# skovaka/UNCALLED

Measured on NVIDIA H100. Metric: reads/sec mapped (E. coli, 4k-sample reads) at 1/2/4/8 H100 vs CPU ref, higher is better.
Workload: dtype f32/f64 events, u32 FM index

## Files before the change

### uncalled_b200/csrc/unc_device.cuh

```cuda
#pragma once
#include "unc_warp.cuh"

typedef uint8_t u8;
typedef uint16_t u16;
typedef uint32_t u32;
typedef int32_t i32;
typedef uint64_t u64;

#define UNC_NKMER 1024
#define UNC_KMASK 0x3FFu
#define UNC_SEED_LEN 22u
#define UNC_NGEN 24u
#define UNC_PATH_MASK 0x3FFFFFu
#define UNC_PATH_TAIL 0x200000u
#define UNC_INVALID 0x80000000u
#define UNC_BLK 32u


struct DevIndex {
    const uint4 *bwt;
    const u32 *sa;
    const u32 *sa_full;
    const uint2 *kmer_range;
    const float *lv_mean, *lv_var2, *lognorm;
// ... 742 lines not shown
#else
#define K2_DYN_FUSE 0u
#endif
#ifdef K2_LEAN_B
#define K2_DYN_PER_CHUNK (44u + K2_DYN_FUSE)
#else
#define K2_DYN_PER_CHUNK (24u + K2_DYN_FUSE)
#endif
#define K2_SMEM_BYTES(maxp) (sizeof(K2Shared) + 16 + (size_t) (((maxp) + 31) / 32) * K2_DYN_PER_CHUNK + 32 + K2_V2_DYN_BYTES)
struct K2Tables {
    uint2 kmer_range[UNC_NKMER];
    float thresh[64];
};
struct K2V2 {
    K2V2Tab t;
    u32 kcnt[UNC_NKMER];
    u32 koff[UNC_NKMER];
    u32 kagg[UNC_NKMER];
    u32 fresh_cand[32], fresh_mask[32], fresh_before[32];
    u32 grab[2];
    u32 n_units;
    u16 mfirst[K2V2_MAX_MERGED];
#if defined(UNC_PHASE_TIMING) && !defined(UNC_EMUL)
    u32 pt_dur[4][K2_MAXSEG];
#endif
};
struct K2Shared {
    K2Tables tb;
    float probs[UNC_NKMER];
    u32 flags[32];
    u32 flags_prev[32];
#ifdef K2_OCC_STAGE
    uint4 occ_stage[K2_MAXSEG * 32 * 5];
#endif
    u32 hist_cur[K2_RB * K2_MAXSEG];
    u32 hist_next[K2_RB * K2_MAXSEG];
    uint2 *agg;
    u64 *pre;
    u32 *bcnt, *ecnt;
    u32 *cmb;
    K2V2 v2;
    unsigned char *v2_stage;
#ifdef K2_DFUSE
    u64 *agg2;
#endif
    u32 bc[8];
    u32 scan_tmp[32];
    u32 n_rows[2];
    u32 verdict[2];
    u32 wk_overflow;
    u32 wl_cnt;
    u32 cnt_blocks, cnt_steps;
    u32 tot_children[2], tot_sources[2];
#ifdef K2_TRK_INLINE
    u32 trk_state[24];
#endif
};

#include "unc_pdqsort.cuh"
#ifdef UNC_EMUL
static unsigned long g_emu_tie_stats[2];
#endif

UNC_DEV void k2_wk_exscan_bins(K2Shared *sh, u32 *src, u32 *dst, u32 wt, u32 nwt) {
    const u32 n = K2_RB * K2_MAXSEG;
    const u32 per = (n + nwt - 1) / nwt;
    const u32 lo = wt * per < n ? wt * per : n, hi = lo + per < n ? lo + per : n;
    u32 sum = 0;
    for (u32 j = lo; j < hi; j++) sum += src[j];
    u32 wtot, woff = w_exscan(sum, &wtot);
    if (w_lane() == 31) sh->scan_tmp[wt >> 5] = wtot;
    c_sync_sub(1, (int) nwt);
#ifdef K2_SCAN2
    u32 run;
    {
        u32 v = (u32) w_lane() < (nwt >> 5) ? sh->scan_tmp[w_lane()] : 0, t;
        u32 e = w_exscan(v, &t);
        run = w_shfl(e, (int) (wt >> 5)) + woff;
    }
#else
    if (wt < 32) {
        u32 v = wt < (nwt >> 5) ? sh->scan_tmp[wt] : 0, t;
        u32 e = w_exscan(v, &t);
        sh->scan_tmp[wt] = e;
    }
    c_sync_sub(1, (int) nwt);
    u32 run = sh->scan_tmp[wt >> 5] + woff;
#endif
    for (u32 j = lo; j < hi; j++) {
        u32 cnt = src[j];
        dst[j] = run;
        src[j] = 0;
        run += cnt;
    }
    c_sync_sub(1, (int) nwt);
}

UNC_DEV void write_source(uint4 *rec, uint2 *hist_e, u32 idx, u32 st, u32 en, u32 kmer, float prob) {
    rec[(size_t) idx * 2] = make_uint4(st, en, kmer | (1u << 16), 1u);
    rec[(size_t) idx * 2 + 1] = make_uint4(f2u(prob), f2u(prob), 0u, 0u);
    hist_e[idx] = make_uint2(f2u(prob), 0xFFFFFFFFu);
}

UNC_DEV u32 unc_event_to_bp(u32 evt_i, bool last, float mean_event_len, float bp_per_samp) {
    float v = f_add(f_mul(f_mul((float) evt_i, mean_event_len), bp_per_samp), (float) (last ? 4 : 0));
    return f_to_u32_x86(v);
// ... 1154 lines not shown
        trk_state_load(sh->trk_state, t1);
        const u32 verdict = sh->trk_state[21], final_event = sh->trk_state[22];
        if (STREAM) {
            DevMapState *ms = B.mstate + B.chan[r];
            ms->t_nb = t1.nb; ms->t_n_alloc = t1.n_alloc; ms->t_n_live = t1.n_live; ms->t_n_lens = t1.n_lens;
            ms->t_top1 = t1.top1; ms->t_top2 = t1.top2; ms->t_overflow = t1.overflow; ms->t_len_sum = t1.len_sum;
            ms->t_max_map[0] = t1.max_map.ren_start; ms->t_max_map[1] = t1.max_map.evt_en; ms->t_max_map[2] = t1.max_map.ref_st;
            ms->t_max_map[3] = t1.max_map.ren_end; ms->t_max_map[4] = t1.max_map.evt_st; ms->t_max_map[5] = t1.max_map.total_len;
            ms->event_i = final_event;
            ms->started = 1;
        }
        unc_k2_write_record(ix, p, B, sh, r, t1, verdict, final_event, ((u64) sh->trk_state[20] << 32) | sh->trk_state[19]);
    }
#else
    if (tid < 32) unc_k2_tracker<STREAM>(ix, p, B, W, sh, r, n_first, n_limit,
                                                              K2_V2_ACTIVE && !EXACT ? (uint4 *) sh->hist_next : nullptr, K2_RB * K2_MAXSEG / 4u);
#ifndef K2_V1
    else if (!EXACT) unc_k2_workers_v2<STREAM, FLAGS>(ix, p, B, W, sh, r, n_first, n_limit);
#endif
    else unc_k2_workers<STREAM, EXACT, FLAGS>(ix, p, B, W, sh, r, n_first, n_limit, epoch_io);
#endif
    c_sync();
    if (STREAM && tid < 32) B.mstate[B.chan[r]].flags[tid] = sh->flags[tid];
    if (!STREAM && FLAGS && B.flags_out && tid < 32) B.flags_out[(size_t) r * 32 + tid] = sh->flags[tid];
}

UNC_DEV bool unc_event0_cand(const DevIndex &ix, const DevParams &p, const DevBatch &B, u32 r, u32 k) {
    if (B.n_events[r] == 0 || p.max_events == 0) return false;
    const float event = f_add(f_mul(B.scale[r], B.events[(size_t) r * B.ev_stride]), B.shift[r]);
    const uint2 kr = ix.kmer_range[k];
    return unc_match_prob(event, d_ldg(ix.lv_mean + k), d_ldg(ix.lv_var2 + k), d_ldg(ix.lognorm + k)) >= ix.thresh[0] &&
           kr.x <= kr.y;
}

UNC_DEV DevWork unc_work_slot(const DevWork &W0, const DevWorkStrides &S, size_t slot) {
    DevWork W;
    W.paths = W0.paths + slot * S.paths;
    W.hist = W0.hist + slot * S.hist;
    W.wlist = W0.wlist + slot * S.cks;
    W.ckey = W0.ckey + slot * S.ckey;
    W.cks = W0.cks + slot * S.cks;
    W.elist = W0.elist + slot * S.elist;
    W.order = W0.order + slot * S.order;
    W.rlist = W0.rlist + slot * S.rlist;
    W.clu = W0.clu + slot * S.clu;
    W.dir = W0.dir + slot * S.dir;
    W.max_blocks = W0.max_blocks;
    W.rl_cap = W0.rl_cap;
    return W;
}

template <bool EXACT = false, bool FLAGS = false>
UNC_DEV void unc_k2_cta_main(const DevIndex &ix, const DevParams &p, const DevBatch &B, const DevWork &W, K2Shared *sh) {
    unc_k2_cta_setup(ix, p, sh);
    u32 epoch = 0;
    for (;;) {
        if (c_tid() == 0) sh->bc[0] = d_atomic_add(B.queue, 1u);
        c_sync();
        u32 r = sh->bc[0];
        c_sync();
        if (r >= B.n_reads) break;
        unc_k2_map_read<false, EXACT, FLAGS>(ix, p, B, W, sh, r, &epoch);
    }
}

template <bool EXACT = false>
UNC_DEV void unc_k2_cta_main_stream(const DevIndex &ix, const DevParams &p, const DevBatch &B, const DevWork &W0,
                                    const DevWorkStrides &S, K2Shared *sh) {
    unc_k2_cta_setup(ix, p, sh);
    u32 epoch = 0;
    for (;;) {
        if (c_tid() == 0) sh->bc[0] = d_atomic_add(B.queue, 1u);
        c_sync();
        u32 r = sh->bc[0];
        c_sync();
        if (r >= B.n_reads) break;
        const DevWork W = unc_work_slot(W0, S, B.chan[r]);
        unc_k2_map_read<true, EXACT, true>(ix, p, B, W, sh, r, &epoch);
    }
}
```

### uncalled_b200/csrc/unc_k2v2.cuh

```cuda
#pragma once

#define K2V2_STAGE_BYTES (K2_CH_SLOTS * 8u + K2_CH_SLOTS)


UNC_DEV void unc_occ2_build_block(const uint4 *bwt, u32 j, uint4 *out) {
    const uint4 *p = bwt + ((size_t) (j >> 1) << 2);
    const uint4 b0 = p[0], b1 = p[1];
    uint4 cnt = make_uint4(b0.x, b0.z, b1.x, b1.z);
    const uint4 lo = p[2], hi = p[3];
    if (j & 1u) {
        const u32 w[4] = {lo.x, lo.y, lo.z, lo.w};
        for (int i = 0; i < 4; i++) {
            const u32 h = w[i] >> 1, m = 0x55555555u;
            const u32 c3 = (u32) d_popc(h & w[i] & m), c2 = (u32) d_popc(h & ~w[i] & m), c1 = (u32) d_popc(~h & w[i] & m);
            cnt.x += 16u - c1 - c2 - c3; cnt.y += c1; cnt.z += c2; cnt.w += c3;
        }
    }
    out[(size_t) j * 2] = cnt;
    out[(size_t) j * 2 + 1] = (j & 1u) ? hi : lo;
}

UNC_DEV void unc_occ2_all(const uint4 cnt, const uint4 sym, u32 p, u32 o[4]) {
    u32 c1 = 0, c2 = 0, c3 = 0;
#pragma unroll
// ... 108 lines not shown
UNC_DEV K2V2Walk k2v2_walk(const uint4 cur, u32 nx, u32 ny, bool a, bool has_next, bool head, bool first, bool use_carry,
                           u32 carry_mx, bool prob_ok, uint2 kr, u32 *mx_last) {
    const int lane = w_lane();
    K2V2Walk r;
    r.dup = has_next && nx == cur.x && ny == cur.y;
    u32 mx = a ? cur.y : 0u;
    bool hd = head || !a;
    for (int d = 1; d < 32; d <<= 1) {
        const u32 omx = w_shfl_up(mx, d), ohd = w_shfl_up(hd ? 1u : 0u, d);
        if (lane >= d && !hd) { mx = omx > mx ? omx : mx; hd = ohd != 0; }
    }
    if (use_carry) mx = mx > carry_mx ? mx : carry_mx;
    *mx_last = w_shfl(mx, 31);
    r.begin_v = a && first && prob_ok && kr.x <= cur.x - 1u;
    r.as = mx + 1u;
    r.ae = has_next ? nx - 1u : kr.y;
    r.after_v = a && !r.dup && prob_ok && r.as <= r.ae;
    r.seed = a && !r.dup && (cur.w & 1u);
    r.m_b = w_ballot(r.begin_v); r.m_a = w_ballot(r.after_v); r.m_seed = w_ballot(r.seed);
    return r;
}

struct K2V2Pack {
    bool a;
    u32 bl;
    u32 start, pos, n;
};
UNC_DEV K2V2Pack k2v2_next_pack(u32 cnt, u32 P, u32 *remaining) {
    const int lane = w_lane();
    const int s = d_ffs(*remaining) - 1;
    const u32 Ps = w_shfl(P, s);
    const bool fits = ((*remaining >> lane) & 1u) && (P + cnt - Ps <= 32u);
    const u32 in_pack = w_ballot(fits);
    *remaining &= ~in_pack;
    const int e = 31 - d_clz(in_pack);
    const u32 T = w_shfl(P + cnt, e) - Ps;
    K2V2Pack k;
    k.a = (u32) lane < T;
    k.bl = (u32) s; k.start = 0;
    u32 m = in_pack;
    while (m) {
        const int b = d_ffs(m) - 1;
        m &= m - 1;
        const u32 sb = w_shfl(P, b) - Ps;
        if ((u32) lane >= sb) { k.bl = (u32) b; k.start = sb; }
    }
    k.pos = (u32) lane - k.start;
    k.n = w_shfl(cnt, (int) k.bl);
    return k;
}
UNC_DEV u32 k2v2_segmask(u32 start, u32 n) { return (n >= 32u ? 0xFFFFFFFFu : ((1u << n) - 1u)) << start; }

UNC_DEV u32 k2v2_slot(u32 rank) { return ((rank & 31u) << 5) | (rank >> 5); }

UNC_DEV u32 k2v2_grab(u32 *counter) {
    u32 g = 0;
    if (w_lane() == 0) g = s_atomic_add(counter, 1u);
    return w_shfl(g, 0);
}

UNC_DEV void k2v2_sort_small(uint4 *keys, u32 n, uint4 *sst) {
    const int lane = w_lane();
    const bool a = (u32) lane < n;
    uint4 k = make_uint4(0, 0, 0, 0);
    if (a) k = keys[lane];
    u32 rnk = 0;
    const u32 kf = k2v2_fkey(k.z), kr_ = k.w >> 14;
    for (u32 j = 0; j < n; j++) {
        const u32 jx = w_shfl(k.x, (int) j), jy = w_shfl(k.y, (int) j), jf = w_shfl(kf, (int) j), jr = w_shfl(kr_, (int) j);
        if (k2v2_less_pre(jx, jy, jf, jr, k.x, k.y, kf, kr_)) rnk++;
    }
    if (a) sst[rnk] = k;
    w_sync();
    if (a) keys[lane] = sst[lane];
    w_sync();
}

struct K2V2Emit {
    uint4 *next; uint2 *hist_e; u32 *onext; uint2 *rlist;
    u32 S0, nc, maxp, n_ended_rows, rl_cap, pos0;
    u32 src_before, seeds_before;
};
template <bool EMIT>
UNC_DEV u32 k2v2_walk_merged(const DevIndex &ix, K2Shared *sh, const uint4 *keys, u32 n, u32 moff, float source_prob,
                             const K2V2Emit &E, u32 *pend_steps, u32 *pend_blocks, uint4 *sst) {
    K2V2 *v2 = &sh->v2;
    const u32 lane = (u32) w_lane();
    u32 nsrc = 0, nseed = 0, prev_sub = 0xFFFFFFFFu, un_st = 1, un_en = 0;
  for (u32 g0 = 0; g0 < n; g0 += 32u) {
    const u32 cnt = n - g0 < 32u ? n - g0 : 32u;
    if (lane < cnt) sst[lane] = keys[g0 + lane];
    if (lane == 0 && g0 + cnt < n) sst[32] = keys[g0 + cnt];
    w_sync();
    if (lane == 0)
    for (u32 j = 0; j < cnt; j++) {
        const u32 i = g0 + j;
        const uint4 cur = sst[j];
        const u32 sub = (cur.w >> 6) & 0xFFu, kmer = v2->t.mk[moff + sub];
        const uint2 kr = sh->tb.kmer_range[kmer];
        const float pk = sh->probs[kmer];
        const bool ok = pk >= source_prob;
        if (sub != prev_sub) {
            if (!EMIT && v2->mfirst[moff + sub] == 0xFFFFu) v2->mfirst[moff + sub] = (u16) nsrc;
            if (ok) {
                if (kr.x <= cur.x - 1u) {
                    const u32 sidx = E.src_before + nsrc;
// ... 20 lines not shown
                src_en = nxt.x - 1u;
                if (un_st <= nxt.y) un_st = nxt.y + 1u;
            }
            if (src_st <= src_en) {
                const u32 sidx = E.src_before + nsrc;
                if (EMIT && E.nc + sidx < E.maxp) {
                    write_source(E.next, E.hist_e, E.S0 + E.nc + sidx, src_st, src_en, kmer, pk);
                    E.onext[E.nc + sidx] = E.S0 + E.nc + sidx;
                }
                nsrc++;
            }
        }
        if (cur.w & 1u) {
            if (EMIT) {
                d_atomic_or(&((u32 *) (E.next + (size_t) rec * 2))[3], 0x80000000u);
                const u32 ri = E.n_ended_rows + E.seeds_before + nseed;
                if (ri < E.rl_cap) E.rlist[ri] = make_uint2(ix.seq_len - unc_sa_lookup(ix, cur.x, pend_steps, pend_blocks), (cur.w >> 1) & 0x1Fu);
                else sh->wk_overflow = 1;
            }
            nseed++;
        }
    }
    w_sync();
  }
    return w_shfl(nsrc | (nseed << 16), 0);
}

UNC_DEV void k2v2_bucket_offsets(K2V2 *v2) {
    const u32 lane = (u32) w_lane();
    u32 sum = 0;
#pragma unroll 1
    for (u32 j = 0; j < 32; j++) sum += v2->kcnt[j * 32u + lane];
    u32 tot, run = w_exscan(sum, &tot);
#pragma unroll 1
    for (u32 j = 0; j < 32; j++) {
        const u32 sl = j * 32u + lane, v = v2->kcnt[sl];
        v2->koff[sl] = run;
        v2->kcnt[sl] = run;
        run += v;
    }
}

template <bool STREAM, bool FLAGS>
UNC_DEV void unc_k2_workers_v2(const DevIndex &ix, const DevParams &p, const DevBatch &B, const DevWork &W,
                               K2Shared *sh, u32 r, u32 n_first, u32 n_limit) {
    const int lane = w_lane();
    const u32 wt = (u32) c_tid() - 32u, nwt = (u32) c_nthreads() - 32u;
    const u32 ww = wt >> 5, nwk = nwt >> 5;
    const K2Tables *tb = &sh->tb;
    K2V2 *v2 = &sh->v2;
    const u32 maxp = p.max_paths;
    const u32 S0 = ((maxp + 31u) >> 5) * K2_CH_SLOTS;
    const size_t gen_recs = (size_t) S0 + maxp;
    const float scale = B.scale[r], shift = B.shift[r];
    const float *events = B.events + (size_t) r * B.ev_stride;
    const float source_prob = tb->thresh[0];
    u64 n_children = 0, n_sources = 0;
    u32 pend_children = 0, pend_sources = 0;
    u32 my_blocks = 0, my_steps = 0, pend_blocks = 0, pend_steps = 0;
    u32 prev_size = 0, gen = 0, event_i = n_first;
    if (STREAM) {
        const DevMapState *ms = B.mstate + B.chan[r];
        if (ms->started) { prev_size = ms->prev_size; gen = ms->gen; }
    }
    const u32 lt = w_lanemask_lt();
    uint2 *stage_r = (uint2 *) (sh->v2_stage + (size_t) ww * K2V2_STAGE_BYTES);
    u8 *stage_m = (u8 *) (stage_r + K2_CH_SLOTS);
    u32 *whist = sh->hist_cur + (size_t) ww * 256u;
    PT_DECL
    PT_WDECL

    for (; event_i < n_limit; event_i++) {
        PT_MARK(9)
        const float event = f_add(f_mul(scale, events[event_i - n_first]), shift);
        PT_MARK(7)

        if (FLAGS && wt < 32u) sh->flags_prev[wt] = sh->flags[wt];
        for (u32 k = wt; k < UNC_NKMER; k += nwt) {
            sh->probs[k] = unc_match_prob(event, d_ldg(ix.lv_mean + k), d_ldg(ix.lv_var2 + k), d_ldg(ix.lognorm + k));
            v2->kcnt[k] = 0; v2->kagg[k] = 0;
        }
        for (u32 j = ww; j < 32; j += nwk) {
            const u32 k = j * 32 + (u32) lane;
            const float pk = unc_match_prob(event, d_ldg(ix.lv_mean + k), d_ldg(ix.lv_var2 + k), d_ldg(ix.lognorm + k));
            const uint2 kr = tb->kmer_range[k];
            const u32 m = w_ballot(pk >= source_prob && kr.x <= kr.y);
            if (lane == 0) v2->fresh_cand[j] = m;
        }
        if (wt == 0) { v2->grab[0] = 0; v2->grab[1] = 0; v2->n_units = 0; }
        if (wt < K2V2_MAX_MERGED) v2->mfirst[wt] = 0xFFFFu;
        PT_MARK(0)
        c_sync_sub(1, (int) nwt);
        PT_FENCE
        PT_MARK(16)

        uint4 *prev = W.paths + (size_t) gen * gen_recs * 2, *next = W.paths + (size_t) (gen ^ 1u) * gen_recs * 2;
        uint2 *hist_e = W.hist + (size_t) (event_i % UNC_NGEN) * gen_recs;
        const u32 *oprev = W.order + (size_t) gen * maxp;
        u32 *onext = W.order + (size_t) (gen ^ 1u) * maxp;
        uint4 *ckA = W.ckey, *ckB = W.ckey + maxp, *cks = W.cks;
        uint2 *rlist = W.rlist + (size_t) (event_i & 1u) * W.rl_cap;

        const u32 nch_prev = (prev_size + 31u) >> 5;
        {
            u32 oi_n = UNC_INVALID, oi_nn = UNC_INVALID; uint4 q0_n = make_uint4(0, 0, 0, 0); uint2 q1_n = make_uint2(0, 0);
            if (ww < nch_prev) {
                const u32 pi = ww * 32u + (u32) lane;
                if (pi < prev_size) oi_n = oprev[pi];
                if (!(oi_n & UNC_INVALID)) { const uint4 *pr = prev + (size_t) oi_n * 2; q0_n = pr[0]; q1_n = *(const uint2 *) (pr + 1); }
            }
            if (ww + nwk < nch_prev) {
                const u32 pi = (ww + nwk) * 32u + (u32) lane;
                if (pi < prev_size) oi_nn = oprev[pi];
                if (!(oi_nn & UNC_INVALID)) d_prefetch(prev + (size_t) oi_nn * 2);
            }
            for (u32 c = ww; c < nch_prev; c += nwk) {
                const u32 oi = oi_n;
                const uint4 q0 = q0_n; const uint2 q1 = q1_n;
                const bool valid = !(oi & UNC_INVALID);
                oi_n = oi_nn;
                if (c + nwk < nch_prev && !(oi_n & UNC_INVALID)) {
                    const uint4 *pr = prev + (size_t) oi_n * 2;
                    q0_n = pr[0]; q1_n = *(const uint2 *) (pr + 1);
                }
                oi_nn = UNC_INVALID;
                if (c + 2u * nwk < nch_prev) {
                    const u32 pi = (c + 2u * nwk) * 32u + (u32) lane;
                    if (pi < prev_size) oi_nn = oprev[pi];
                    if (!(oi_nn & UNC_INVALID)) d_prefetch(prev + (size_t) oi_nn * 2);
                }
                const u32 st = q0.x, en = q0.y, kmer = q0.z & UNC_KMASK, plen = (q0.z >> 16) & 0xFFu, stays = (q0.z >> 24) & 0xFFu;
                const u32 moves = q0.w & UNC_PATH_MASK, sa_checked = q0.w >> 31;
                u32 want = 0, cmask = 0;
                if (valid) {
                    const float thr = tb->thresh[32 + d_clz(en - st + 1u)];
                    if (stays < p.max_consec_stay && sh->probs[kmer] >= thr) cmask = 1u;
#pragma unroll
                    for (u32 b = 0; b < 4; b++)
                        if (!(sh->probs[((kmer << 2) & UNC_KMASK) | b] < thr)) want |= 1u << b;
                }
                if (cmask) stage_r[(u32) lane * 5u] = make_uint2(st, en);
                if (want) {
                    const u32 k0 = st - 1u, l0 = en;
                    const u32 kk = k0 - (k0 >= ix.primary), ll = l0 - (l0 >= ix.primary);
                    const bool l_is_end = (l0 == ix.seq_len);
                    const uint4 *bk = ix.occ2 + ((size_t) (kk >> 6) << 1);
                    const uint4 kc = d_ldg(bk), ks = d_ldg(bk + 1);
                    uint4 lc = kc, ls = ks;
                    if (!l_is_end && (ll >> 6) != (kk >> 6)) {
                        const uint4 *bl = ix.occ2 + ((size_t) (ll >> 6) << 1);
                        lc = d_ldg(bl); ls = d_ldg(bl + 1);
                    }
                    pend_blocks += 1u + ((!l_is_end && (ll >> 7) != (kk >> 7)) ? 1u : 0u);
                    u32 ok[4], ol[4];
                    unc_occ2_all(kc, ks, kk & 63u, ok);
                    unc_occ2_all(lc, ls, ll & 63u, ol);
                    if (l_is_end) { ol[0] = ix.L2[1] - ix.L2[0]; ol[1] = ix.L2[2] - ix.L2[1]; ol[2] = ix.L2[3] - ix.L2[2]; ol[3] = ix.L2[4] - ix.L2[3]; }
// ... 34 lines not shown
                    const u32 pz = w_shfl(q0.z, L), pw = w_shfl(q0.w, L), pC = w_shfl(q1.y, L), poi = w_shfl(oi, L);
                    if (act) {
                        const u32 pk = pz & UNC_KMASK, ppl = (pz >> 16) & 0xFFu, pst = (pz >> 24) & 0xFFu;
                        const u32 ckm = j == 0 ? pk : (((pk << 2) & UNC_KMASK) | (j - 1u));
                        const float pb = sh->probs[ckm];
                        const u32 move = j > 0 ? 1u : 0u;
                        const u32 nlen = ppl + (ppl < UNC_SEED_LEN ? 1u : 0u);
                        u32 nmoves = (((pw & UNC_PATH_MASK) << 1) | move) & UNC_PATH_MASK;
                        const u32 nstays = move ? 0u : pst + 1u;
                        const float newC = f_add(u2f(pC), pb);
                        const u32 ci = c * K2_CH_SLOTS + t;
                        float sp = 0.0f;
                        bool seedable = false;
                        if (ppl == UNC_SEED_LEN) {
                            nmoves |= UNC_PATH_TAIL;
                            W.wlist[s_atomic_add(&sh->wl_cnt, 1u)] = make_uint4(ci, poi, f2u(newC), nmoves);
                        } else {
                            sp = f_div(newC, (float) nlen);
                            const u32 cmc = (u32) d_popc(nmoves);
                            seedable = nlen == UNC_SEED_LEN && sp >= p.min_seed_prob && rg.x == rg.y && (nmoves & 1u) &&
                                       (float) ((nlen - cmc) & 0xFFu) <= f_mul(p.max_stay_frac, 22.0f);
                        }
                        const u32 spb = f2u(sp);
                        next[(size_t) ci * 2] = make_uint4(rg.x, rg.y, ckm | (nlen << 16) | (nstays << 24), nmoves | (pw & 0x80000000u));
                        next[(size_t) ci * 2 + 1] = make_uint4(spb, f2u(newC), 0u, 0u);
                        hist_e[ci] = make_uint2(f2u(newC), poi);
                        cks[ci] = make_uint4(rg.x, rg.y, spb, ckm | (seedable ? 1u << 10 : 0u) | ((u32) d_popc(nmoves) << 11));
                        s_atomic_add(&v2->kcnt[v2->t.kslot[ckm]], 1u);
                    }
                }
                if (c + nwk < nch_prev && !(oi_n & UNC_INVALID)) {
                    const u32 k0n = q0_n.x - 1u;
                    d_prefetch(ix.occ2 + ((size_t) ((k0n - (k0n >= ix.primary)) >> 6) << 1));
                }
                w_sync();
            }
        }
        PT_MARK(1)
        c_sync_sub(1, (int) nwt);
        PT_FENCE
        PT_MARK(17)
        if (ww == 0) {
            {
                const u32 per = (nch_prev + 31u) >> 5, c_lo = (u32) lane * per, c_hi = c_lo + per < nch_prev ? c_lo + per : nch_prev;
                u32 sum = 0;
#pragma unroll 1
                for (u32 c = c_lo; c < c_hi; c++) sum += sh->bcnt[c];
                u32 tot, run = w_exscan(sum, &tot);
#pragma unroll 1
                for (u32 c = c_lo; c < c_hi; c++) { const u32 v = sh->bcnt[c]; sh->bcnt[c] = run; run += v; }
                if (lane == 0) sh->bc[2] = tot;
            }
            w_sync();
            u32 rows = 0;
            for (u32 i0 = 0; i0 < nch_prev; i0 += 32) {
                u32 ec = i0 + (u32) lane < nch_prev ? sh->ecnt[i0 + lane] : 0u;
                u32 m = w_ballot(ec != 0);
                while (m) {
                    int l = d_ffs(m) - 1;
                    m &= m - 1;
                    u32 c = i0 + (u32) l, n = w_shfl(ec, l), base = sh->bcnt[c];
                    for (u32 j = 0; j < n; j++) {
                        uint4 e = W.elist[(size_t) c * 32 + j];
                        if (base + e.w < maxp) {
                            u32 len = e.y - e.x + 1u;
                            if (rows + len <= W.rl_cap) {
                                for (u32 i = (u32) lane; i < len; i += 32) rlist[rows + i] = make_uint2(e.x + i, e.z | 0x100u);
                            } else sh->wk_overflow = 1;
                            rows += len;
                        }
                    }
                }
            }
            if (lane == 0) sh->bc[3] = rows;
        }
        if (ww == nwk - 1u) {
            k2v2_bucket_offsets(v2);
        }
        if (ww != 0 || nwk == 1) {
            const u32 bt = nwk == 1 ? wt : wt - 32u, nbt = nwk == 1 ? nwt : nwt - 32u;
            const u32 nwl = *(volatile u32 *) &sh->wl_cnt;
            for (u32 i = bt; i < nwl; i += nbt) {
                uint4 w = W.wlist[i];
                u32 idx = w.y;
                for (u32 j = 1; j <= 21; j++)
                    idx = W.hist[(size_t) ((event_i + UNC_NGEN - j) % UNC_NGEN) * gen_recs + idx].y;
                float oldC = u2f(W.hist[(size_t) ((event_i + UNC_NGEN - 22u) % UNC_NGEN) * gen_recs + idx].x);
                float sp = f_div(f_sub(u2f(w.z), oldC), 22.0f);
                uint4 key = cks[w.x];
                u32 cmc = (u32) d_popc(w.w);
                bool seedable = sp >= p.min_seed_prob && key.x == key.y && (w.w & 1u) &&
                                (float) ((UNC_SEED_LEN - cmc) & 0xFFu) <= f_mul(p.max_stay_frac, 22.0f);
                key.z = f2u(sp);
                if (seedable) key.w |= 1u << 10;
                cks[w.x] = key;
                next[(size_t) w.x * 2 + 1].x = f2u(sp);
            }
        }
        PT_MARK(10)
        c_sync_sub(1, (int) nwt);
        PT_FENCE
        PT_MARK(26)
        if (wt == 0) sh->wl_cnt = 0;
        const u32 nc_total = nch_prev ? sh->bc[2] : 0u;
        const u32 nc = nc_total < maxp ? nc_total : maxp;
        if (nc_total > maxp) {
            for (u32 c = ww; c < nch_prev; c += nwk) {
                const u32 base = sh->bcnt[c], end = c + 1 < nch_prev ? sh->bcnt[c + 1] : nc_total;
                if (end <= nc) continue;
                for (u32 i = (base < nc ? nc - base : 0u) + (u32) lane; base + i < end; i += 32)
                    s_atomic_add(&v2->kagg[v2->t.kslot[cks[(size_t) c * K2_CH_SLOTS + i].w & UNC_KMASK]], 1u);
            }
            c_sync_sub(1, (int) nwt);
            if (ww == 0) {
                const u32 l = (u32) lane;
#pragma unroll 1
                for (u32 j = 0; j < 32; j++) {
                    const u32 sl = j * 32u + l;
                    const u32 nxt = j < 31u ? v2->koff[sl + 32u] : (l < 31u ? v2->koff[l + 1u] : nc_total);
                    v2->kcnt[sl] = nxt - v2->koff[sl] - v2->kagg[sl];
                    v2->kagg[sl] = 0;
                }
                w_sync();
                k2v2_bucket_offsets(v2);
            }
            c_sync_sub(1, (int) nwt);
        }
        PT_MARK(12)
        u32 n_rows = sh->bc[3];
        if (n_rows > W.rl_cap) n_rows = W.rl_cap;
        const u32 n_ended_rows = n_rows;
        pend_children = nc;

        if (nc > 0) {
            uint4 kpre = make_uint4(0, 0, 0, 0);
            if (ww < nch_prev) {
                const u32 b0 = sh->bcnt[ww], e0 = ww + 1 < nch_prev ? sh->bcnt[ww + 1] : nc_total;
                if (b0 + (u32) lane < e0 && b0 + (u32) lane < nc) kpre = cks[(size_t) ww * K2_CH_SLOTS + (u32) lane];
            }
            for (u32 c = ww; c < nch_prev; c += nwk) {
                const u32 base = sh->bcnt[c];
                if (base >= nc) break;
                const u32 end = c + 1 < nch_prev ? sh->bcnt[c + 1] : nc_total;
                const uint4 kcur = kpre;
                if (c + nwk < nch_prev) {
                    const u32 bn = sh->bcnt[c + nwk], en = c + nwk + 1 < nch_prev ? sh->bcnt[c + nwk + 1] : nc_total;
                    if (bn + (u32) lane < en && bn + (u32) lane < nc) kpre = cks[(size_t) (c + nwk) * K2_CH_SLOTS + (u32) lane];
                }
                for (u32 i = (u32) lane; base + i < end && base + i < nc; i += 32) {
                    const u32 ci = c * K2_CH_SLOTS + i;
                    uint4 key = i < 32u ? kcur : cks[ci];
                    const u32 km = key.w & UNC_KMASK;
                    const u32 bk = v2->t.kslot[km];
                    key.w = ((key.w >> 10) & 0x3Fu) | ((u32) v2->t.ksub[km] << 6) | (ci << 14);
                    ckA[s_atomic_add(&v2->kcnt[bk], 1u)] = key;
                }
            }
            PT_MARK(2)
            c_sync_sub(1, (int) nwt);
            PT_FENCE
            PT_MARK(18)
            PT_WB

            uint4 *csum = W.elist;
            for (;;) {
                const u32 gi = k2v2_grab(&v2->grab[0]);
                if (gi >= 96u) break;
                const u32 grp = gi & 31u;
                const u32 sl = (u32) lane * 32u + grp;
                const u32 bo = v2->koff[sl], bn = v2->kcnt[sl] - bo;
                const u32 meta = v2->t.gmeta[grp * 32u + (u32) lane];
                if (gi < 64u) {
                    const bool huge_sweep = gi < 32u;
                    u32 todo_m = huge_sweep ? w_ballot(meta != 0 && bn > 0) : 0u;
                    while (todo_m) {
                        const int l = d_ffs(todo_m) - 1;
                        todo_m &= todo_m - 1;
                        const u32 o = w_shfl(bo, l), n = w_shfl(bn, l), moff = w_shfl(meta, l) >> 8;
                        if (n <= 32u) k2v2_sort_small(ckA + o, n, (uint4 *) stage_r);
                        else {
                            u32 lo = 0xFFFFFFFFu, hi = 0;
                            for (u32 g = (u32) lane; g < n; g += 32u) { const u32 x = ckA[o + g].x; lo = x < lo ? x : lo; hi = x > hi ? x : hi; }
                            hi = w_max(hi);
                            lo = ~w_max(~lo);
                            k2v2_sort_big(ckA, ckB, o, n, lo, 32u - (u32) d_clz(hi - lo), whist);
                        }
                        {
                            K2V2Emit E;
                            E.src_before = 0; E.seeds_before = 0;
                            const u32 agg = k2v2_walk_merged<false>(ix, sh, ckA + o, n, moff, source_prob, E, &pend_steps, &pend_blocks, (uint4 *) stage_r);
                            if (lane == 0) v2->kagg[(u32) l * 32u + grp] = agg;
                        }
                    }
                    u32 todo = w_ballot(meta == 0 && (huge_sweep ? bn > 256u : (bn > 32u && bn <= 256u)));
                    while (todo) {
                        const int l = d_ffs(todo) - 1;
                        todo &= todo - 1;
                        const u32 o = w_shfl(bo, l), n = w_shfl(bn, l);
                        const u32 kmer = v2->t.gkmer[grp * 32u + (u32) l];
                        u32 ubase = 0;
                        if (lane == 0) ubase = s_atomic_add(&v2->n_units, (n + 31u) >> 5);
                        ubase = w_shfl(ubase, 0);
                        const uint2 kr = tb->kmer_range[kmer];
                        const bool prob_ok = sh->probs[kmer] >= source_prob;
                        u32 lo = 0xFFFFFFFFu, hi = 0;
                        for (u32 g = (u32) lane; g < n; g += 32u) { const u32 x = ckA[o + g].x; lo = x < lo ? x : lo; hi = x > hi ? x : hi; }
                        hi = w_max(hi);
                        lo = ~w_max(~lo);
                        k2v2_sort_big(ckA, ckB, o, n, lo, 32u - (u32) d_clz(hi - lo), whist);
                        u32 carry_mx = 0, n_src = 0, n_seed = 0;
                        for (u32 g0 = 0; g0 < n; g0 += 32u) {
                            const u32 g = g0 + (u32) lane;
                            const bool a = g < n, has_next = g + 1u < n;
                            uint4 cur = make_uint4(0, 0, 0, 0); u32 nx = 0, ny = 0;
                            if (a) cur = ckA[o + g];
                            if (has_next) { const uint4 t = ckA[o + g + 1u]; nx = t.x; ny = t.y; }
                            if (lane == 0) csum[ubase + (g0 >> 5)] = make_uint4(carry_mx, n_src, n_seed, ((u32) l * 32u + grp) | ((g0 >> 5) << 10));
// ... 42 lines not shown
                    }
                }
            }
            PT_WE(1)
            PT_MARK(3)
            c_sync_sub(1, (int) nwt);
            PT_FENCE
            PT_MARK(19)
            PT_WR(1, 15, 20)
        }

        if (ww == 0) {
            u32 sum = 0;
#pragma unroll 1
            for (u32 j = 0; j < 32; j++) sum += v2->kagg[j * 32u + (u32) lane];
            u32 ts, tq;
            const u32 es = w_exscan(sum & 0xFFFFu, &ts), eq = w_exscan(sum >> 16, &tq);
            u32 run = es | (eq << 16);
#pragma unroll 1
            for (u32 j = 0; j < 32; j++) {
                const u32 sl = j * 32u + (u32) lane, v = v2->kagg[sl];
                v2->kagg[sl] = run;
                if (nc > 0 && v2->kcnt[sl] != v2->koff[sl]) {
                    const u32 meta = v2->t.gmeta[(u32) lane * 32u + j];
                    if (meta == 0) {
                        const u32 kmer = v2->t.gkmer[(u32) lane * 32u + j];
                        if (sh->probs[kmer] >= source_prob && nc + (run & 0xFFFFu) < maxp) s_atomic_or(&sh->flags[kmer >> 5], 1u << (kmer & 31u));
                    } else {
                        for (u32 m = 0; m < (meta & 0xFFu); m++) {
                            const u32 f = v2->mfirst[(meta >> 8) + m], kmer = v2->t.mk[(meta >> 8) + m];
                            if (f != 0xFFFFu && sh->probs[kmer] >= source_prob && nc + (run & 0xFFFFu) + f < maxp)
                                s_atomic_or(&sh->flags[kmer >> 5], 1u << (kmer & 31u));
                        }
                    }
                }
                run = ((run & 0xFFFFu) + (v & 0xFFFFu)) | (((run >> 16) + (v >> 16)) << 16);
            }
            w_sync();
            const u32 tot_src = ts;
            const u32 ns_added = nc + tot_src > maxp ? maxp - nc : tot_src;
            const u32 nn0 = nc + ns_added;
            const u32 my_mask = v2->fresh_cand[lane] & ~sh->flags[lane];
            u32 tot_add;
            const u32 my_pre = w_exscan((u32) d_popc(my_mask), &tot_add);
            v2->fresh_mask[lane] = my_mask;
            v2->fresh_before[lane] = nn0 + my_pre;
            if (lane == 0) {
                sh->bc[1] = nn0 + tot_add < maxp ? nn0 + tot_add : maxp;
                sh->bc[6] = tq;
            }
        }
        if (ww != 0 || nwk == 1) {
            const u32 bt = nwk == 1 ? wt : wt - 32u, nbt = nwk == 1 ? nwt : nwt - 32u;
            for (u32 i = bt; i < n_ended_rows; i += nbt) {
                uint2 e = rlist[i];
                e.x = ix.seq_len - unc_sa_lookup(ix, e.x, &pend_steps, &pend_blocks);
                rlist[i] = e;
            }
        }
        PT_MARK(11)
        c_sync_sub(1, (int) nwt);
        PT_FENCE
        PT_MARK(27)
        PT_WB
        const u32 n_child_seeds = nc > 0 ? sh->bc[6] : 0u;
        n_rows = n_ended_rows + n_child_seeds;
        if (n_rows > W.rl_cap) n_rows = W.rl_cap;

        if (nc > 0) {
            const uint4 *csum = W.elist;
            const u32 n_units = *(volatile u32 *) &v2->n_units;
            for (;;) {
                const u32 gi = k2v2_grab(&v2->grab[1]);
                if (gi >= n_units + 32u) break;
                if (gi < n_units) {
                    const uint4 u = csum[gi];
                    const u32 sl_u = u.w & 1023u, g0 = (u.w >> 10) << 5;
                    const u32 o = v2->koff[sl_u], n = v2->kcnt[sl_u] - o, pre = v2->kagg[sl_u];
                    const u32 kmer = v2->t.gkmer[((sl_u & 31u) << 5) | (sl_u >> 5)];
                    const uint2 kr = tb->kmer_range[kmer];
                    const float pkm = sh->probs[kmer];
                    const bool prob_ok = pkm >= source_prob;
                    const u32 pos = g0 + (u32) lane;
                    const bool a = pos < n, has_next = pos + 1u < n;
                    uint4 cur = make_uint4(0, 0, 0, 0);
                    if (a) cur = ckA[o + pos];
                    u32 nx = w_shfl_down(cur.x, 1), ny = w_shfl_down(cur.y, 1);
                    if (lane == 31 && has_next) { const uint4 t = ckA[o + pos + 1u]; nx = t.x; ny = t.y; }
                    u32 mxo;
                    const K2V2Walk wk = k2v2_walk(cur, nx, ny, a, has_next, pos == 0, pos == 0, g0 != 0, u.x, prob_ok, kr, &mxo);
                    const u32 sidx = (pre & 0xFFFFu) + u.y + (u32) d_popc(wk.m_b & lt) + (u32) d_popc(wk.m_a & lt);
                    if (wk.begin_v && nc + sidx < maxp) {
                        write_source(next, hist_e, S0 + nc + sidx, kr.x, cur.x - 1u, kmer, pkm);
                        onext[nc + sidx] = S0 + nc + sidx;
                    }
                    const u32 sidx2 = sidx + (wk.begin_v ? 1u : 0u);
                    if (wk.after_v && nc + sidx2 < maxp) {
                        write_source(next, hist_e, S0 + nc + sidx2, wk.as, wk.ae, kmer, pkm);
                        onext[nc + sidx2] = S0 + nc + sidx2;
                    }
                    const u32 rec = cur.w >> 14;
                    if (a) onext[o + pos] = rec | (wk.dup ? UNC_INVALID : 0u);
                    if (wk.seed) {
                        d_atomic_or(&((u32 *) (next + (size_t) rec * 2))[3], 0x80000000u);
                        const u32 ri = n_ended_rows + (pre >> 16) + u.z + (u32) d_popc(wk.m_seed & lt);
                        if (ri < W.rl_cap)
                            rlist[ri] = make_uint2(ix.seq_len - unc_sa_lookup(ix, cur.x, &pend_steps, &pend_blocks), (cur.w >> 1) & 0x1Fu);
                        else sh->wk_overflow = 1;
                    }
                    continue;
                }
                const u32 grp = gi - n_units;
                const u32 sl = (u32) lane * 32u + grp;
                const u32 bo = v2->koff[sl], bn = v2->kcnt[sl] - bo, bpre = v2->kagg[sl];
                const u32 meta = v2->t.gmeta[grp * 32u + (u32) lane];
                u32 todo_m = w_ballot(meta != 0 && bn > 0);
                while (todo_m) {
                    const int l = d_ffs(todo_m) - 1;
                    todo_m &= todo_m - 1;
                    {
                        const u32 o_m = w_shfl(bo, l), n_m = w_shfl(bn, l), pre_m = w_shfl(bpre, l), mt_m = w_shfl(meta, l);
                        K2V2Emit E;
                        E.next = next; E.hist_e = hist_e; E.onext = onext; E.rlist = rlist;
                        E.S0 = S0; E.nc = nc; E.maxp = maxp; E.n_ended_rows = n_ended_rows; E.rl_cap = W.rl_cap; E.pos0 = o_m;
                        E.src_before = pre_m & 0xFFFFu; E.seeds_before = pre_m >> 16;
                        k2v2_walk_merged<true>(ix, sh, ckA + o_m, n_m, mt_m >> 8, source_prob, E, &pend_steps, &pend_blocks, (uint4 *) stage_r);
                    }
                }
                const u32 cnt = (bn > 0 && bn <= 32u && meta == 0) ? bn : 0u;
                u32 tot;
                const u32 P = w_exscan(cnt, &tot);
                u32 remaining = w_ballot(cnt != 0);
                while (remaining) {
                    const K2V2Pack pk = k2v2_next_pack(cnt, P, &remaining);
                    const u32 kmer = v2->t.gkmer[grp * 32u + pk.bl];
                    const uint2 kr = tb->kmer_range[kmer];
                    const float pkm = sh->probs[kmer];
                    const bool prob_ok = pkm >= source_prob;
                    const u32 pre = w_shfl(bpre, (int) pk.bl), o = w_shfl(bo, (int) pk.bl);
                    uint4 cur = make_uint4(0, 0, 0, 0);
                    if (pk.a) cur = ckA[o + pk.pos];
                    const u32 nx = w_shfl_down(cur.x, 1), ny = w_shfl_down(cur.y, 1);
                    u32 mxo;
                    const K2V2Walk wk = k2v2_walk(cur, nx, ny, pk.a, pk.a && pk.pos + 1u < pk.n, pk.pos == 0, pk.pos == 0, false, 0u, prob_ok,
                                                  kr, &mxo);
                    const u32 sm = k2v2_segmask(pk.start, pk.n);
                    const u32 sidx = (pre & 0xFFFFu) + (u32) d_popc(wk.m_b & lt & sm) + (u32) d_popc(wk.m_a & lt & sm);
                    if (wk.begin_v && nc + sidx < maxp) {
                        write_source(next, hist_e, S0 + nc + sidx, kr.x, cur.x - 1u, kmer, pkm);
                        onext[nc + sidx] = S0 + nc + sidx;
                    }
                    const u32 sidx2 = sidx + (wk.begin_v ? 1u : 0u);
                    if (wk.after_v && nc + sidx2 < maxp) {
                        write_source(next, hist_e, S0 + nc + sidx2, wk.as, wk.ae, kmer, pkm);
                        onext[nc + sidx2] = S0 + nc + sidx2;
                    }
                    const u32 rec = cur.w >> 14;
                    if (pk.a) onext[o + pk.pos] = rec | (wk.dup ? UNC_INVALID : 0u);
                    if (wk.seed) {
                        d_atomic_or(&((u32 *) (next + (size_t) rec * 2))[3], 0x80000000u);
                        const u32 ri = n_ended_rows + (pre >> 16) + (u32) d_popc(wk.m_seed & lt & sm);
                        if (ri < W.rl_cap)
                            rlist[ri] = make_uint2(ix.seq_len - unc_sa_lookup(ix, cur.x, &pend_steps, &pend_blocks), (cur.w >> 1) & 0x1Fu);
                        else sh->wk_overflow = 1;
                    }
                }
            }
        }
        PT_WE(2)
        for (u32 j = ww; j < 32; j += nwk) {
            const u32 before = v2->fresh_before[j];
            if (before >= maxp) continue;
            const u32 k = j * 32 + (u32) lane;
            const u32 fw = sh->flags[j];
            u32 m_add = v2->fresh_mask[j];
            const u32 room = maxp - before;
            u32 visited = 0xFFFFFFFFu;
            if ((u32) d_popc(m_add) >= room) {
                u32 mm = m_add;
                for (u32 q = 1; q < room; q++) mm &= mm - 1;
                int last = d_ffs(mm) - 1;
                visited = last == 31 ? 0xFFFFFFFFu : ((2u << last) - 1u);
                m_add &= visited;
            }
            const u32 rank = (u32) d_popc(m_add & lt);
            if ((m_add >> lane) & 1u) {
                const uint2 kr = tb->kmer_range[k];
                write_source(next, hist_e, S0 + before + rank, kr.x, kr.y, k, sh->probs[k]);
                onext[before + rank] = S0 + before + rank;
            }
            w_sync();
            if (lane == 0) sh->flags[j] = fw & ~visited;
        }
        if (wt == 0) *(volatile u32 *) &sh->n_rows[event_i & 1u] = n_rows;
        PT_WARR(3)
        PT_MARK(5)
        c_sync();
        PT_WREL(0)
        PT_FENCE
        PT_MARK(6)
        PT_WR(2, 21, 22)
        PT_WLAG(3, 23, 24)
        PT_WLAG(0, 13, 14)
        PT_WTRK(3, 25)
        const u32 nn = sh->bc[1];
        pend_sources = nn - nc;
        const u32 v = event_i > n_first ? *(volatile u32 *) &sh->verdict[(event_i - 1u) & 1u] : 0u;
        if (v) {
            if (FLAGS && wt < 32u) sh->flags[wt] = sh->flags_prev[wt];
            break;
        }
        n_children += pend_children; n_sources += pend_sources;
        my_blocks += pend_blocks; my_steps += pend_steps;
        pend_children = pend_sources = pend_blocks = pend_steps = 0;
        prev_size = nn;
        gen ^= 1u;
        PT_MARK(8)
    }
    if (STREAM && wt == 0) { DevMapState *ms = B.mstate + B.chan[r]; ms->prev_size = prev_size; ms->gen = gen; }
    PT_FLUSH(B, r)
    for (int d = 16; d > 0; d >>= 1) { my_blocks += w_shfl(my_blocks, lane ^ d); my_steps += w_shfl(my_steps, lane ^ d); }
    if (lane == 0) { s_atomic_add(&sh->cnt_blocks, my_blocks); s_atomic_add(&sh->cnt_steps, my_steps); }
    if (wt == 0) {
        sh->tot_children[0] = (u32) n_children; sh->tot_children[1] = (u32) (n_children >> 32);
        sh->tot_sources[0] = (u32) n_sources; sh->tot_sources[1] = (u32) (n_sources >> 32);
    }
    c_sync();
}
```

Baseline: 4950.

## Cut register pressure in k2 worker loop by moving state to shared memory

Several long-lived values in the k2 v2 worker loop are no longer held in registers across the whole event loop. The DevWork struct now lives in shared memory, and the 64-bit child and source totals are accumulated in shared memory by thread 0. Per-generation pointers are recomputed inside each phase's scope instead of being held live, and the history chain walk uses a decrementing slot index with unroll disabled. The aim is fewer live registers, which could avoid spills or allow higher occupancy, at the cost of extra shared-memory loads and repeated address arithmetic.

```diff
diff --git a/uncalled_b200/csrc/unc_device.cuh b/uncalled_b200/csrc/unc_device.cuh
--- a/uncalled_b200/csrc/unc_device.cuh
+++ b/uncalled_b200/csrc/unc_device.cuh
@@ -818,6 +818,7 @@
     u32 wl_cnt;
     u32 cnt_blocks, cnt_steps;
     u32 tot_children[2], tot_sources[2];
+    DevWork work;
 #ifdef K2_TRK_INLINE
     u32 trk_state[24];
 #endif
@@ -2078,6 +2079,7 @@
 
 template <bool EXACT = false, bool FLAGS = false>
 UNC_DEV void unc_k2_cta_main(const DevIndex &ix, const DevParams &p, const DevBatch &B, const DevWork &W, K2Shared *sh) {
+    if (c_tid() == 0) sh->work = W;
     unc_k2_cta_setup(ix, p, sh);
     u32 epoch = 0;
     for (;;) {
@@ -2086,7 +2088,7 @@
         u32 r = sh->bc[0];
         c_sync();
         if (r >= B.n_reads) break;
-        unc_k2_map_read<false, EXACT, FLAGS>(ix, p, B, W, sh, r, &epoch);
+        unc_k2_map_read<false, EXACT, FLAGS>(ix, p, B, sh->work, sh, r, &epoch);
     }
 }
 
@@ -2101,7 +2103,7 @@
         u32 r = sh->bc[0];
         c_sync();
         if (r >= B.n_reads) break;
-        const DevWork W = unc_work_slot(W0, S, B.chan[r]);
-        unc_k2_map_read<true, EXACT, true>(ix, p, B, W, sh, r, &epoch);
-    }
-}
+        if (c_tid() == 0) sh->work = unc_work_slot(W0, S, B.chan[r]);
+        unc_k2_map_read<true, EXACT, true>(ix, p, B, sh->work, sh, r, &epoch);
+    }
+}
diff --git a/uncalled_b200/csrc/unc_k2v2.cuh b/uncalled_b200/csrc/unc_k2v2.cuh
--- a/uncalled_b200/csrc/unc_k2v2.cuh
+++ b/uncalled_b200/csrc/unc_k2v2.cuh
@@ -184,6 +184,16 @@
 UNC_DEV u32 k2v2_segmask(u32 start, u32 n) { return (n >= 32u ? 0xFFFFFFFFu : ((1u << n) - 1u)) << start; }
 
 UNC_DEV u32 k2v2_slot(u32 rank) { return ((rank & 31u) << 5) | (rank >> 5); }
+
+UNC_DEV uint2 *k2v2_stage(K2Shared *sh, u32 ww) {
+    const u32 off = (u32) (sh->v2_stage - (unsigned char *) sh) + ww * K2V2_STAGE_BYTES;
+    return (uint2 *) ((unsigned char *) sh + off);
+}
+
+UNC_DEV void k2v2_add64(u32 *w, u32 v) {
+    const u64 s = (((u64) w[1] << 32) | w[0]) + v;
+    w[0] = (u32) s; w[1] = (u32) (s >> 32);
+}
 
 UNC_DEV u32 k2v2_grab(u32 *counter) {
     u32 g = 0;
@@ -310,27 +320,21 @@
     const u32 maxp = p.max_paths;
     const u32 S0 = ((maxp + 31u) >> 5) * K2_CH_SLOTS;
     const size_t gen_recs = (size_t) S0 + maxp;
-    const float scale = B.scale[r], shift = B.shift[r];
-    const float *events = B.events + (size_t) r * B.ev_stride;
     const float source_prob = tb->thresh[0];
-    u64 n_children = 0, n_sources = 0;
-    u32 pend_children = 0, pend_sources = 0;
     u32 my_blocks = 0, my_steps = 0, pend_blocks = 0, pend_steps = 0;
     u32 prev_size = 0, gen = 0, event_i = n_first;
     if (STREAM) {
         const DevMapState *ms = B.mstate + B.chan[r];
         if (ms->started) { prev_size = ms->prev_size; gen = ms->gen; }
     }
+    if (wt == 0) { sh->tot_children[0] = sh->tot_children[1] = 0; sh->tot_sources[0] = sh->tot_sources[1] = 0; }
     const u32 lt = w_lanemask_lt();
-    uint2 *stage_r = (uint2 *) (sh->v2_stage + (size_t) ww * K2V2_STAGE_BYTES);
-    u8 *stage_m = (u8 *) (stage_r + K2_CH_SLOTS);
-    u32 *whist = sh->hist_cur + (size_t) ww * 256u;
     PT_DECL
     PT_WDECL
 
     for (; event_i < n_limit; event_i++) {
         PT_MARK(9)
-        const float event = f_add(f_mul(scale, events[event_i - n_first]), shift);
+        const float event = f_add(f_mul(B.scale[r], B.events[(size_t) r * B.ev_stride + (event_i - n_first)]), B.shift[r]);
         PT_MARK(7)
 
         if (FLAGS && wt < 32u) sh->flags_prev[wt] = sh->flags[wt];
@@ -352,15 +356,15 @@
         PT_FENCE
         PT_MARK(16)
 
-        uint4 *prev = W.paths + (size_t) gen * gen_recs * 2, *next = W.paths + (size_t) (gen ^ 1u) * gen_recs * 2;
-        uint2 *hist_e = W.hist + (size_t) (event_i % UNC_NGEN) * gen_recs;
-        const u32 *oprev = W.order + (size_t) gen * maxp;
-        u32 *onext = W.order + (size_t) (gen ^ 1u) * maxp;
-        uint4 *ckA = W.ckey, *ckB = W.ckey + maxp, *cks = W.cks;
-        uint2 *rlist = W.rlist + (size_t) (event_i & 1u) * W.rl_cap;
 
         const u32 nch_prev = (prev_size + 31u) >> 5;
         {
+            const uint4 *prev = W.paths + (size_t) gen * gen_recs * 2;
+            uint4 *next = W.paths + (size_t) (gen ^ 1u) * gen_recs * 2, *cks = W.cks;
+            uint2 *hist_e = W.hist + (size_t) (event_i % UNC_NGEN) * gen_recs;
+            const u32 *oprev = W.order + (size_t) gen * maxp;
+            uint2 *stage_r = k2v2_stage(sh, ww);
+            u8 *stage_m = (u8 *) (stage_r + K2_CH_SLOTS);
             u32 oi_n = UNC_INVALID, oi_nn = UNC_INVALID; uint4 q0_n = make_uint4(0, 0, 0, 0); uint2 q1_n = make_uint2(0, 0);
             if (ww < nch_prev) {
                 const u32 pi = ww * 32u + (u32) lane;
@@ -501,6 +505,7 @@
                 if (lane == 0) sh->bc[2] = tot;
             }
             w_sync();
+            uint2 *rlist = W.rlist + (size_t) (event_i & 1u) * W.rl_cap;
             u32 rows = 0;
             for (u32 i0 = 0; i0 < nch_prev; i0 += 32) {
                 u32 ec = i0 + (u32) lane < nch_prev ? sh->ecnt[i0 + lane] : 0u;
@@ -529,12 +534,19 @@
         if (ww != 0 || nwk == 1) {
             const u32 bt = nwk == 1 ? wt : wt - 32u, nbt = nwk == 1 ? nwt : nwt - 32u;
             const u32 nwl = *(volatile u32 *) &sh->wl_cnt;
+            uint4 *next = W.paths + (size_t) (gen ^ 1u) * gen_recs * 2, *cks = W.cks;
+            const uint2 *hist = W.hist;
+            const u32 recs = (u32) gen_recs, s_e = event_i % UNC_NGEN;
             for (u32 i = bt; i < nwl; i += nbt) {
                 uint4 w = W.wlist[i];
-                u32 idx = w.y;
-                for (u32 j = 1; j <= 21; j++)
-                    idx = W.hist[(size_t) ((event_i + UNC_NGEN - j) % UNC_NGEN) * gen_recs + idx].y;
-                float oldC = u2f(W.hist[(size_t) ((event_i + UNC_NGEN - 22u) % UNC_NGEN) * gen_recs + idx].x);
+                u32 idx = w.y, s = s_e;
+#pragma unroll 1
+                for (u32 j = 0; j < 21u; j++) {
+                    s = s ? s - 1u : UNC_NGEN - 1u;
+                    idx = hist[s * recs + idx].y;
+                }
+                s = s ? s - 1u : UNC_NGEN - 1u;
+                float oldC = u2f(hist[s * recs + idx].x);
                 float sp = f_div(f_sub(u2f(w.z), oldC), 22.0f);
                 uint4 key = cks[w.x];
                 u32 cmc = (u32) d_popc(w.w);
@@ -558,7 +570,7 @@
                 const u32 base = sh->bcnt[c], end = c + 1 < nch_prev ? sh->bcnt[c + 1] : nc_total;
                 if (end <= nc) continue;
                 for (u32 i = (base < nc ? nc - base : 0u) + (u32) lane; base + i < end; i += 32)
-                    s_atomic_add(&v2->kagg[v2->t.kslot[cks[(size_t) c * K2_CH_SLOTS + i].w & UNC_KMASK]], 1u);
+                    s_atomic_add(&v2->kagg[v2->t.kslot[W.cks[(size_t) c * K2_CH_SLOTS + i].w & UNC_KMASK]], 1u);
             }
             c_sync_sub(1, (int) nwt);
             if (ww == 0) {
@@ -579,9 +591,11 @@
         u32 n_rows = sh->bc[3];
         if (n_rows > W.rl_cap) n_rows = W.rl_cap;
         const u32 n_ended_rows = n_rows;
-        pend_children = nc;
 
         if (nc > 0) {
+          {
+            uint4 *ckA = W.ckey;
+            const uint4 *cks = W.cks;
             uint4 kpre = make_uint4(0, 0, 0, 0);
             if (ww < nch_prev) {
                 const u32 b0 = sh->bcnt[ww], e0 = ww + 1 < nch_prev ? sh->bcnt[ww + 1] : nc_total;
@@ -605,6 +619,7 @@
                     ckA[s_atomic_add(&v2->kcnt[bk], 1u)] = key;
                 }
             }
+          }
             PT_MARK(2)
             c_sync_sub(1, (int) nwt);
             PT_FENCE
@@ -612,6 +627,9 @@
             PT_WB
 
             uint4 *csum = W.elist;
+            uint4 *ckA = W.ckey, *ckB = W.ckey + maxp;
+            uint2 *stage_r = k2v2_stage(sh, ww);
+            u32 *whist = sh->hist_cur + (size_t) ww * 256u;
             for (;;) {
                 const u32 gi = k2v2_grab(&v2->grab[0]);
                 if (gi >= 96u) break;
@@ -760,6 +778,7 @@
         }
         if (ww != 0 || nwk == 1) {
             const u32 bt = nwk == 1 ? wt : wt - 32u, nbt = nwk == 1 ? nwt : nwt - 32u;
+            uint2 *rlist = W.rlist + (size_t) (event_i & 1u) * W.rl_cap;
             for (u32 i = bt; i < n_ended_rows; i += nbt) {
                 uint2 e = rlist[i];
                 e.x = ix.seq_len - unc_sa_lookup(ix, e.x, &pend_steps, &pend_blocks);
@@ -776,7 +795,12 @@
         if (n_rows > W.rl_cap) n_rows = W.rl_cap;
 
         if (nc > 0) {
-            const uint4 *csum = W.elist;
+            const uint4 *csum = W.elist, *ckA = W.ckey;
+            uint4 *next = W.paths + (size_t) (gen ^ 1u) * gen_recs * 2;
+            uint2 *hist_e = W.hist + (size_t) (event_i % UNC_NGEN) * gen_recs;
+            u32 *onext = W.order + (size_t) (gen ^ 1u) * maxp;
+            uint2 *rlist = W.rlist + (size_t) (event_i & 1u) * W.rl_cap;
+            uint2 *stage_r = k2v2_stage(sh, ww);
             const u32 n_units = *(volatile u32 *) &v2->n_units;
             for (;;) {
                 const u32 gi = k2v2_grab(&v2->grab[1]);
@@ -876,6 +900,9 @@
             }
         }
         PT_WE(2)
+        uint4 *next = W.paths + (size_t) (gen ^ 1u) * gen_recs * 2;
+        uint2 *hist_e = W.hist + (size_t) (event_i % UNC_NGEN) * gen_recs;
+        u32 *onext = W.order + (size_t) (gen ^ 1u) * maxp;
         for (u32 j = ww; j < 32; j += nwk) {
             const u32 before = v2->fresh_before[j];
             if (before >= maxp) continue;
@@ -912,15 +939,14 @@
         PT_WLAG(0, 13, 14)
         PT_WTRK(3, 25)
         const u32 nn = sh->bc[1];
-        pend_sources = nn - nc;
         const u32 v = event_i > n_first ? *(volatile u32 *) &sh->verdict[(event_i - 1u) & 1u] : 0u;
         if (v) {
             if (FLAGS && wt < 32u) sh->flags[wt] = sh->flags_prev[wt];
             break;
         }
-        n_children += pend_children; n_sources += pend_sources;
+        if (wt == 0) { k2v2_add64(sh->tot_children, nc); k2v2_add64(sh->tot_sources, nn - nc); }
         my_blocks += pend_blocks; my_steps += pend_steps;
-        pend_children = pend_sources = pend_blocks = pend_steps = 0;
+        pend_blocks = pend_steps = 0;
         prev_size = nn;
         gen ^= 1u;
         PT_MARK(8)
@@ -929,9 +955,5 @@
     PT_FLUSH(B, r)
     for (int d = 16; d > 0; d >>= 1) { my_blocks += w_shfl(my_blocks, lane ^ d); my_steps += w_shfl(my_steps, lane ^ d); }
     if (lane == 0) { s_atomic_add(&sh->cnt_blocks, my_blocks); s_atomic_add(&sh->cnt_steps, my_steps); }
-    if (wt == 0) {
-        sh->tot_children[0] = (u32) n_children; sh->tot_children[1] = (u32) (n_children >> 32);
-        sh->tot_sources[0] = (u32) n_sources; sh->tot_sources[1] = (u32) (n_sources >> 32);
-    }
     c_sync();
 }
```

Measured after the change: 5261, median of 6. +6.3%, better.
